# facebookarchive/Surround360

Measured on AMD Instinct MI355X. Metric: stereo-equirect frames/sec at 8K, 17-cam rig, higher is better.
Workload: dtype f32

## Files before the change

surround360_amd/csrc/flow_kernels.hip:

```cpp
#include "flow_kernels.hpp"

#include <algorithm>
#include <cmath>
#include <cstdlib>
#include <stdexcept>

#include "devmath.hpp"

namespace s360 {

typedef float f4a8 __attribute__((ext_vector_type(4), aligned(8)));

__global__ __launch_bounds__(256) void k_resize_cubic_u8c4(const uchar4* __restrict__ src, int sw, int sh,
                                                           size_t sbs, uchar4* __restrict__ dst, int dw, int dh,
                                                           size_t dbs, double scx, double scy,
                                                           const uchar4* const* __restrict__ src_tab) {
  __shared__ int s_sx[32], s_sy[8];
  __shared__ short s_ax[32][4], s_ay[8][4];
  const int tid = threadIdx.y * blockDim.x + threadIdx.x;
  if (tid < 40) {
    const bool col = tid < 32;
    const int k = col ? tid : tid - 32;
    const int d = col ? min((int)(blockIdx.x * 32 + k), dw - 1) : min((int)(blockIdx.y * 8 + k), dh - 1);
    int s0;
// ... 211 lines not shown
  for (int j = 0; j < 4; ++j) {
    int sx;
    float cb[4];
    resize_coord(min(dx0 + j, dw - 1), scx, &sx, &f);
    cubic_coeffs(f, cb);
    int a[4];
#pragma unroll
    for (int k = 0; k < 4; ++k) a[k] = sat_s16(cv_round(cb[k] * 2048.f));
    c[j] = sx - 1 - bx0;
    w01[j] = __builtin_bit_cast(s16x2, (unsigned)(a[0] & 0xffff) | ((unsigned)a[1] << 16));
    w23[j] = __builtin_bit_cast(s16x2, (unsigned)(a[2] & 0xffff) | ((unsigned)a[3] << 16));
  }
  int r0, ay[4];
  {
    int sy;
    float cb[4];
    resize_coord(min(dy, dh - 1), scy, &sy, &f);
    cubic_coeffs(f, cb);
#pragma unroll
    for (int k = 0; k < 4; ++k) ay[k] = sat_s16(cv_round(cb[k] * 2048.f));
    r0 = sy - 1 - by0;
  }
  __syncthreads();
  if (dx0 >= dw || dy >= dh) return;
  const float scale = 1.f / (2048 * 2048);
  const float b0 = (float)ay[0] * scale, b1 = (float)ay[1] * scale, b2 = (float)ay[2] * scale, b3 = (float)ay[3] * scale;
  auto pixel = [&](int j, const unsigned (&p)[4][4]) -> unsigned {
    const bool sse = dx0 + j < (dw & ~1);
    unsigned o = 0;
#pragma unroll
    for (int ch = 0; ch < 4; ++ch) {
      const unsigned sel = 0x0c040c00u + ch * 0x00010001u;
      int hh[4];
#pragma unroll
      for (int r = 0; r < 4; ++r) {
        const s16x2 lo = __builtin_bit_cast(s16x2, __builtin_amdgcn_perm(p[r][1], p[r][0], sel));
        const s16x2 hi = __builtin_bit_cast(s16x2, __builtin_amdgcn_perm(p[r][3], p[r][2], sel));
        hh[r] = __builtin_amdgcn_sdot2(lo, w01[j], 0, false);
        hh[r] = __builtin_amdgcn_sdot2(hi, w23[j], hh[r], false);
      }
      int v;
      if (sse) {
        float s = (float)hh[0] * b0;
        s = s + (float)hh[1] * b1;
        s = s + (float)hh[2] * b2;
        s = s + (float)hh[3] * b3;
        v = cv_round(s);
      } else {
        v = (__mul24(hh[0], ay[0]) + __mul24(hh[1], ay[1]) + __mul24(hh[2], ay[2]) + __mul24(hh[3], ay[3]) + (1 << 21)) >> 22;
      }
      o |= (unsigned)sat_u8(v) << (8 * ch);
    }
    return o;
  };
  unsigned o[4];
  if (c[1] == c[0] + 2 && c[2] == c[0] + 4 && c[3] == c[0] + 6 && (c[0] & 3) == 0) {
    unsigned t[4][10];
#pragma unroll
    for (int r = 0; r < 4; ++r) {
      const unsigned* row = &s_box[r0 + r][c[0]];
      const u32x4 q0 = *reinterpret_cast<const u32x4*>(row), q1 = *reinterpret_cast<const u32x4*>(row + 4);
      typedef unsigned u32x2 __attribute__((ext_vector_type(2)));
      const u32x2 q2 = *reinterpret_cast<const u32x2*>(row + 8);
      t[r][0] = q0.x; t[r][1] = q0.y; t[r][2] = q0.z; t[r][3] = q0.w;
      t[r][4] = q1.x; t[r][5] = q1.y; t[r][6] = q1.z; t[r][7] = q1.w;
      t[r][8] = q2.x; t[r][9] = q2.y;
    }
#pragma unroll
    for (int j = 0; j < 4; ++j) {
      unsigned p[4][4];
#pragma unroll
      for (int r = 0; r < 4; ++r)
#pragma unroll
        for (int k = 0; k < 4; ++k) p[r][k] = t[r][2 * j + k];
      o[j] = pixel(j, p);
    }
  } else {
#pragma unroll
    for (int j = 0; j < 4; ++j) {
      unsigned p[4][4];
#pragma unroll
      for (int r = 0; r < 4; ++r)
#pragma unroll
        for (int k = 0; k < 4; ++k) p[r][k] = s_box[r0 + r][c[j] + k];
      o[j] = pixel(j, p);
    }
  }
  const size_t off = (size_t)dy * dw + dx0;
  const bool whole = dx0 + 3 < dw;
  if (dst) {
    unsigned* Dr = reinterpret_cast<unsigned*>(dst + dbs * blockIdx.z) + off;
    if (whole) {
      *reinterpret_cast<u32x4a4*>(Dr) = u32x4a4{o[0], o[1], o[2], o[3]};
    } else {
#pragma unroll
      for (int j = 0; j < 4; ++j)
        if (dx0 + j < dw) Dr[j] = o[j];
    }
  }
  if (gray) {
    const float inv255 = (float)(1.0 / 255.0);
    float g[4], a[4];
#pragma unroll
    for (int j = 0; j < 4; ++j) {
      const int gi = (int)((o[j] & 0xff) * 1868 + ((o[j] >> 8) & 0xff) * 9617 + ((o[j] >> 16) & 0xff) * 4899 + (1 << 13)) >> 14;
      g[j] = (float)gi * inv255;
      a[j] = (float)(o[j] >> 24) * inv255;
    }
    float* Gr = gray + pbs * blockIdx.z + off;
    float* Ar = alpha + pbs * blockIdx.z + off;
    if (whole) {
      *reinterpret_cast<f32x4a4*>(Gr) = f32x4a4{g[0], g[1], g[2], g[3]};
      *reinterpret_cast<f32x4a4*>(Ar) = f32x4a4{a[0], a[1], a[2], a[3]};
    } else {
#pragma unroll
      for (int j = 0; j < 4; ++j)
        if (dx0 + j < dw) { Gr[j] = g[j]; Ar[j] = a[j]; }
    }
  }
}

__global__ __launch_bounds__(256) void k_gray_alpha(const uchar4* __restrict__ src, size_t n, size_t sbs,
                                                    float* __restrict__ gray, float* __restrict__ alpha,
                                                    size_t pbs) {
  const size_t i = (size_t)blockIdx.x * blockDim.x + threadIdx.x;
  if (i >= n) return;
  const uchar4 p = src[sbs * blockIdx.z + i];
  const float inv255 = (float)(1.0 / 255.0);
  const int g = (p.x * 1868 + p.y * 9617 + p.z * 4899 + (1 << 13)) >> 14;
  gray[pbs * blockIdx.z + i] = (float)g * inv255;
  alpha[pbs * blockIdx.z + i] = (float)p.w * inv255;
}

__global__ __launch_bounds__(256) void k_motion(const uchar4* __restrict__ cur, const uchar4* __restrict__ prev,
                                                size_t n, size_t sbs, float* __restrict__ motion, size_t pbs) {
  const size_t i = (size_t)blockIdx.x * blockDim.x + threadIdx.x;
  if (i >= n) return;
  const uchar4 a = cur[sbs * blockIdx.z + i], b = prev[sbs * blockIdx.z + i];
  const double s = fabs((double)((int)a.x - (int)b.x)) + fabs((double)((int)a.y - (int)b.y)) +
                   fabs((double)((int)a.z - (int)b.z));
  motion[pbs * blockIdx.z + i] = (float)(s / (double)(255.0f * 3.0f));
}

#ifdef S360_WAVE_EMULATION
unsigned long long g_known_stats[2];
#define S360_KSTAT(i) __atomic_fetch_add(&g_known_stats[i], 1ull, __ATOMIC_RELAXED)
#endif
struct UpSrc {
  int sw, sh;
  size_t sbs;
  double scx, scy;
  float post_scale;
};
template <int R, int CN, int EPI, int SRC, int SB_TW = 64, int SB_TH = 16, int NT = 256>
__global__ __launch_bounds__(NT) void k_sepblur(const float* __restrict__ src, float* __restrict__ dst, int w, int h,
                                                 size_t bs , BlurTaps taps,
                                                 const float* __restrict__ A, FlowIdx idx,
                                                 const float2* __restrict__ Gp, void* __restrict__ recv,
                                                 float* const* __restrict__ dst_tab, UpSrc up,
                                                 unsigned* __restrict__ rowflags, int known_result) {
  constexpr int IW = SB_TW + 2 * R, IH = SB_TH + 2 * R;
  constexpr int IWP = IW | 1;
  __shared__ __attribute__((aligned(8))) float s_in[IH][IWP][CN];
  __shared__ __attribute__((aligned(8))) float s_mid[IH][SB_TW + 1][CN];
  const int tid = threadIdx.y * blockDim.x + threadIdx.x;
  const TileId tile = xcd_tile();
  const int tx0 = tile.x * SB_TW, ty0 = tile.y * SB_TH;
  const int vecEnd = ((w * CN) / 8) * 8;
  constexpr int kColTasks = SB_TW * (SB_TH / 4);
  static_assert(EPI == 0 || kColTasks <= NT, "one column task per thread when the epilogue is prefetched");
  float pa0[4] = {0.f, 0.f, 0.f, 0.f}, pa1[4] = {0.f, 0.f, 0.f, 0.f}, pm[4] = {0.f, 0.f, 0.f, 0.f};
  float2 pg[4];
  if (EPI != 0 && tid < kColTasks) {
    const int lx = tid % SB_TW, ly0 = (tid / SB_TW) * 4, gx = tx0 + lx;
    const size_t b0 = bs * idx.i0[tile.z], b1 = bs * idx.i1[tile.z];
#pragma unroll
    for (int o = 0; o < 4; ++o) {
      const int gy = ty0 + ly0 + o;
      pg[o] = make_float2(0.f, 0.f);
      if (gx < w && gy < h) {
        const size_t off = (size_t)gy * w + gx;
        pa0[o] = A[b0 + off];
        pa1[o] = A[b1 + off];
        if (EPI == 3) pg[o] = Gp[b0 + off];
        if (EPI == 4) {
          pg[o] = Gp[bs * tile.z + off];
          pm[o] = static_cast<const float*>(recv)[b1 + off];
        }
      }
    }
  }
  src += (SRC == 2 ? up.sbs * CN : bs * (SRC == 1 ? 1 : CN)) * tile.z;
  constexpr int LW = (IW + 7) & ~7;
  constexpr bool kColumnWalk = (NT % LW) == 0;
  const int lxc = tid % LW, lyc = tid / LW;
  const int gxc = reflect101(tx0 - R + (lxc < IW ? lxc : 0), w);
  constexpr int kLdStep = kColumnWalk ? NT / LW : NT, kLdEnd = kColumnWalk ? IH : IH * IW;
  constexpr int kLdIters = (kLdEnd + kLdStep - 1) / kLdStep;
  float ld[kLdIters][CN];
#pragma unroll
  for (int it = 0; it < kLdIters; ++it) {
    const int i = min((kColumnWalk ? lyc : tid) + it * kLdStep, kLdEnd - 1);
    const int ly = kColumnWalk ? i : i / IW, lx = kColumnWalk ? min(lxc, IW - 1) : i - ly * IW;
    const int gy = reflect101(ty0 - R + ly, h), gx = kColumnWalk ? gxc : reflect101(tx0 - R + lx, w);
    if (SRC == 2) {
      int sx, sy;
      float fx, fy;
      resize_coord(gx, up.scx, &sx, &fx);
      if (sx < 0) { fx = 0; sx = 0; }
      if (sx >= up.sw - 1) { fx = 0; sx = up.sw - 1; }
      resize_coord(gy, up.scy, &sy, &fy);
      const float* S0 = src + (size_t)clip_idx(sy, up.sh) * up.sw * CN;
      const float* S1 = src + (size_t)clip_idx(sy + 1, up.sh) * up.sw * CN;
      const float b0 = 1.f - fy, b1 = fy;
#pragma unroll
      for (int k = 0; k < CN; ++k) {
        float h0, h1;
        if (sx >= up.sw - 1) {
          h0 = S0[sx * CN + k] * 1.0f;
          h1 = S1[sx * CN + k] * 1.0f;
        } else {
          const float a0 = 1.f - fx, a1 = fx;
          h0 = S0[sx * CN + k] * a0 + S0[(sx + 1) * CN + k] * a1;
          h1 = S1[sx * CN + k] * a0 + S1[(sx + 1) * CN + k] * a1;
        }
        float v = h0 * b0 + h1 * b1;
        v *= up.post_scale;
        ld[it][k] = v;
      }
    } else if (SRC == 1) {
      const float* r0 = src + (size_t)gy * w;
      ld[it][0] = r0[min(gx + 1, w - 1)] - r0[max(gx - 1, 0)];
      ld[it][CN - 1] = src[(size_t)min(gy + 1, h - 1) * w + gx] - src[(size_t)max(gy - 1, 0) * w + gx];
    } else if (CN == 2) {
      const float2 v = *reinterpret_cast<const float2*>(src + ((size_t)gy * w + gx) * CN);
      ld[it][0] = v.x;
      ld[it][CN - 1] = v.y;
    } else {
      ld[it][0] = src[(size_t)gy * w + gx];
    }
  }
#pragma unroll
  for (int it = 0; it < kLdIters; ++it) {
    const int i = (kColumnWalk ? lyc : tid) + it * kLdStep;
    if (i >= kLdEnd || (kColumnWalk && lxc >= IW)) continue;
    const int ly = kColumnWalk ? i : i / IW, lx = kColumnWalk ? lxc : i - ly * IW;
    if (CN == 2) *reinterpret_cast<float2*>(&s_in[ly][lx][0]) = make_float2(ld[it][0], ld[it][CN - 1]);
    else s_in[ly][lx][0] = ld[it][0];
  }
  if constexpr (EPI == 2 || EPI == 3) {
    __shared__ int s_vote[NT / 64];
    bool none = true;
#pragma unroll
    for (int o = 0; o < 4; ++o) none &= !(pa0[o] > 0.9f && pa1[o] > 0.9f);
    s_vote[tid >> 6] = __ballot(!none) == 0ull;
    __syncthreads();
    int v = known_result != 0;
#pragma unroll
    for (int q = 0; q < NT / 64; ++q) v &= s_vote[q];
    const bool known = __builtin_amdgcn_readfirstlane(v) != 0;
#ifdef S360_WAVE_EMULATION
    if (tid == 0) S360_KSTAT(known ? 0 : 1);
#endif
    if (known) {
      if (tid < kColTasks) {
        const int lx = tid % SB_TW, ly0 = (tid / SB_TW) * 4, gx = tx0 + lx;
#pragma unroll
        for (int o = 0; o < 4; ++o) {
          const int gy = ty0 + ly0 + o;
          if (gx >= w || gy >= h) continue;
          const size_t off = (size_t)gy * w + gx;
          if (EPI == 2) static_cast<float2*>(recv)[bs * tile.z + off] = make_float2(__int_as_float(0x7fc00000), 0.0f);
          else static_cast<float4*>(recv)[bs * tile.z + off] = make_float4(__int_as_float(0x7fc00000), pg[o].y, 0.0f, 0.0f);
        }
      }
      return;
    }
  } else {
    __syncthreads();
  }
  for (int t = tid; t < IH * (SB_TW / 4); t += NT) {
    const int ly = t % IH, lx0 = (t / IH) * 4;
    float v[CN][4 + 2 * R];
#pragma unroll
    for (int j = 0; j < 4 + 2 * R; ++j) {
      if (CN == 2) {
        const float2 p = *reinterpret_cast<const float2*>(&s_in[ly][lx0 + j][0]);
        v[0][j] = p.x;
        v[CN - 1][j] = p.y;
      } else {
        v[0][j] = s_in[ly][lx0 + j][0];
      }
    }
#pragma unroll
    for (int o = 0; o < 4; ++o) {
      float acc[CN];
#pragma unroll
      for (int k = 0; k < CN; ++k) {
        if (R <= 2) {
          acc[k] = taps.k[0] * v[k][o + R];
#pragma unroll
          for (int j = 1; j <= R; ++j) acc[k] += taps.k[j] * (v[k][o + R + j] + v[k][o + R - j]);
        } else {
          acc[k] = ((tx0 + lx0 + o) * CN + k < vecEnd) ? 0.0f : -0.0f;
#pragma unroll
          for (int j = 0; j <= 2 * R; ++j) acc[k] += taps.k[j < R ? R - j : j - R] * v[k][o + j];
        }
      }
      if (CN == 2) *reinterpret_cast<float2*>(&s_mid[ly][lx0 + o][0]) = make_float2(acc[0], acc[CN - 1]);
      else s_mid[ly][lx0 + o][0] = acc[0];
    }
  }
  __syncthreads();
  dst = dst_tab ? dst_tab[tile.z] : dst + bs * CN * tile.z;
  for (int t = tid; t < SB_TW * (SB_TH / 4); t += NT) {
    const int lx = t % SB_TW, ly0 = (t / SB_TW) * 4;
    const int gx = tx0 + lx;
    float outv[4][CN];
    {
      float v[CN][4 + 2 * R];
#pragma unroll
      for (int j = 0; j < 4 + 2 * R; ++j) {
        if (CN == 2) {
          const float2 p = *reinterpret_cast<const float2*>(&s_mid[ly0 + j][lx][0]);
          v[0][j] = p.x;
          v[CN - 1][j] = p.y;
        } else {
          v[0][j] = s_mid[ly0 + j][lx][0];
        }
      }
      if (CN == 2) {
        typedef float f32x2 __attribute__((ext_vector_type(2)));
        f32x2 p[4 + 2 * R];
#pragma unroll
        for (int j = 0; j < 4 + 2 * R; ++j) p[j] = f32x2{v[0][j], v[CN - 1][j]};
#pragma unroll
        for (int o = 0; o < 4; ++o) {
          f32x2 acc = taps.k[0] * p[o + R] + 0.0f;
#pragma unroll
          for (int j = 1; j <= R; ++j) acc += taps.k[j] * (p[o + R + j] + p[o + R - j]);
          outv[o][0] = acc.x;
          outv[o][CN - 1] = acc.y;
        }
      } else {
#pragma unroll
        for (int k = 0; k < CN; ++k)
#pragma unroll
          for (int o = 0; o < 4; ++o) {
            float acc = taps.k[0] * v[k][o + R] + 0.0f;
#pragma unroll
            for (int j = 1; j <= R; ++j) acc += taps.k[j] * (v[k][o + R + j] + v[k][o + R - j]);
            outv[o][k] = acc;
          }
      }
    }
    if (gx >= w) continue;
#pragma unroll
    for (int o = 0; o < 4; ++o) {
      const int gy = ty0 + ly0 + o;
      if (gy >= h) continue;
      const size_t off = (size_t)gy * w + gx;
      if (EPI == 1 || EPI == 4) {
        const float cc = 1.0f - pa0[o] * pa1[o];
#pragma unroll
        for (int k = 0; k < CN; ++k) outv[o][k] = cc * outv[o][k] + (1.0f - cc) * s_in[ly0 + o + R][lx + R][k];
      }
      if (EPI == 4) {
        const float wgt = 1.0f - pm[o];
        const float px = pg[o].x * up.post_scale, py = pg[o].y * up.post_scale;
        outv[o][0] = outv[o][0] * (1.0f - wgt) + px * wgt;
        outv[o][CN - 1] = outv[o][CN - 1] * (1.0f - wgt) + py * wgt;
      }
      if (EPI == 2 || EPI == 3) {
        const bool upd = pa0[o] > 0.9f && pa1[o] > 0.9f;
        if (EPI == 2)
          static_cast<float2*>(recv)[bs * tile.z + off] = make_float2(upd ? outv[o][0] : __int_as_float(0x7fc00000), outv[o][CN - 1]);
        else
          static_cast<float4*>(recv)[bs * tile.z + off] = make_float4(upd ? pg[o].x : __int_as_float(0x7fc00000), pg[o].y, outv[o][0], outv[o][CN - 1]);
        if (rowflags && upd) rowflags[(size_t)tile.z * h + gy] = 0u;
      } else {
#pragma unroll
        for (int k = 0; k < CN; ++k) dst[off * CN + k] = outv[o][k];
      }
    }
  }
}

constexpr int UB_TW = 64, UB_TH = 16, UB_IW = UB_TW + 2, UB_IH = UB_TH + 2, UB_IWP = UB_IW | 1, UB_BW = 40, UB_BH = 14;
constexpr int UB_IN_FLOATS = UB_IH * UB_IWP * 2, UB_MID_FLOATS = UB_IH * (UB_TW + 1) * 2, UB_H_FLOATS = UB_BH * UB_IW * 2;
static_assert(UB_BH * UB_BW * 2 <= UB_IN_FLOATS, "the source box shares the input tile's storage");
static_assert(UB_H_FLOATS + 2 * UB_IW + 3 * UB_IH <= UB_MID_FLOATS, "horizontal pass + tables share the row-pass result's storage");
bool upscale_blur_tiled_fits(int sw, int sh, int dw, int dh) {
  const double scx = 1.0 / ((double)dw / (double)sw), scy = 1.0 / ((double)dh / (double)sh);
  return 2 * (long long)dw <= 5 * (long long)sw && 2 * (long long)dh <= 5 * (long long)sh && (int)std::ceil((UB_IW - 1) * scx) + 3 <= UB_BW && (int)std::ceil((UB_IH - 1) * scy) + 3 <= UB_BH;
}
__global__ __launch_bounds__(256) void k_upscale_blur_tiled(const float2* __restrict__ src, float* __restrict__ dst, int w, int h,
                                                            size_t bs, BlurTaps taps, float* const* __restrict__ dst_tab,
                                                            UpSrc up) {
  __shared__ __attribute__((aligned(16))) float s_raw[UB_IN_FLOATS + UB_MID_FLOATS];
  float2(*s_in)[UB_IWP] = reinterpret_cast<float2(*)[UB_IWP]>(s_raw);
  float2(*s_mid)[UB_TW + 1] = reinterpret_cast<float2(*)[UB_TW + 1]>(s_raw + UB_IN_FLOATS);
  float2(*s_box)[UB_BW] = reinterpret_cast<float2(*)[UB_BW]>(s_raw);
  float2(*s_h)[UB_IW] = reinterpret_cast<float2(*)[UB_IW]>(s_raw + UB_IN_FLOATS);
  int* s_sx = reinterpret_cast<int*>(s_raw + UB_IN_FLOATS + UB_H_FLOATS);
  float* s_fx = reinterpret_cast<float*>(s_sx + UB_IW);
  int* s_r0 = s_sx + 2 * UB_IW;
  int* s_r1 = s_r0 + UB_IH;
  float* s_fy = reinterpret_cast<float*>(s_r1 + UB_IH);
  const int tid = threadIdx.x;
  const TileId tile = xcd_tile();
  const int tx0 = tile.x * UB_TW, ty0 = tile.y * UB_TH;
  const int nvx = min(UB_TW, w - tx0), nvy = min(UB_TH, h - ty0);
  src += up.sbs * tile.z;
  if (tid < UB_IW) {
    int sx;
    float fx;
    resize_coord(reflect101(tx0 - 1 + min(tid, nvx + 1), w), up.scx, &sx, &fx);
    if (sx < 0) { fx = 0; sx = 0; }
    if (sx >= up.sw - 1) { fx = 0; sx = up.sw - 1; }
    s_sx[tid] = sx;
    s_fx[tid] = fx;
  } else if (tid >= 128 && tid < 128 + UB_IH) {
    const int ly = tid - 128;
    int sy;
    float fy;
    resize_coord(reflect101(ty0 - 1 + min(ly, nvy + 1), h), up.scy, &sy, &fy);
    s_r0[ly] = clip_idx(sy, up.sh);
    s_r1[ly] = clip_idx(sy + 1, up.sh);
    s_fy[ly] = fy;
  }
  __syncthreads();
  const int bx0 = min(s_sx[0], s_sx[1]), by0 = min(s_r0[0], s_r0[1]);
  const int bx1 = min(max(s_sx[nvx], s_sx[nvx + 1]) + 1, up.sw - 1), by1 = max(s_r1[nvy], s_r1[nvy + 1]);
  const int nbw = clip_idx(bx1 - bx0, UB_BW) + 1, nbh = clip_idx(by1 - by0, UB_BH) + 1;
  {
    constexpr int kIters = (UB_BW * UB_BH + 255) / 256;
    float2 ld[kIters];
#pragma unroll
    for (int it = 0; it < kIters; ++it) {
      const int i = tid + it * 256;
      const int r = min(i / UB_BW, nbh - 1), c = min(i % UB_BW, nbw - 1);
      ld[it] = src[(size_t)min(by0 + r, up.sh - 1) * up.sw + min(bx0 + c, up.sw - 1)];
    }
#pragma unroll
    for (int it = 0; it < kIters; ++it) {
      const int i = tid + it * 256;
      const int r = i / UB_BW, c = i % UB_BW;
      if (r < nbh && c < nbw) s_box[r][c] = ld[it];
    }
  }
  __syncthreads();
  for (int t = tid; t < nbh * UB_IW; t += 256) {
    const int r = t / UB_IW, c = t - r * UB_IW;
    const int sx = s_sx[c], cx = clip_idx(sx - bx0, UB_BW);
    const float2 p0 = s_box[r][cx];
    float2 hv;
    if (sx >= up.sw - 1) {
      hv.x = p0.x * 1.0f;
      hv.y = p0.y * 1.0f;
    } else {
      const float fx = s_fx[c];
      const float a0 = 1.f - fx, a1 = fx;
      const float2 p1 = s_box[r][min(cx + 1, UB_BW - 1)];
      hv.x = p0.x * a0 + p1.x * a1;
      hv.y = p0.y * a0 + p1.y * a1;
    }
    s_h[r][c] = hv;
  }
  __syncthreads();
  for (int t = tid; t < UB_IH * UB_IW; t += 256) {
    const int ly = t / UB_IW, lx = t - ly * UB_IW;
    const float fy = s_fy[ly];
    const float b0 = 1.f - fy, b1 = fy;
    const float2 h0 = s_h[clip_idx(s_r0[ly] - by0, UB_BH)][lx], h1 = s_h[clip_idx(s_r1[ly] - by0, UB_BH)][lx];
    float vx = h0.x * b0 + h1.x * b1, vy = h0.y * b0 + h1.y * b1;
    vx *= up.post_scale;
    vy *= up.post_scale;
    s_in[ly][lx] = make_float2(vx, vy);
  }
  __syncthreads();
  typedef float f32x2 __attribute__((ext_vector_type(2)));
  for (int t = tid; t < UB_IH * (UB_TW / 4); t += 256) {
    const int ly = t % UB_IH, lx0 = (t / UB_IH) * 4;
    float2 v[6];
#pragma unroll
    for (int j = 0; j < 6; ++j) v[j] = s_in[ly][lx0 + j];
#pragma unroll
    for (int o = 0; o < 4; ++o) {
      float2 acc;
      acc.x = taps.k[0] * v[o + 1].x;
      acc.x += taps.k[1] * (v[o + 2].x + v[o].x);
      acc.y = taps.k[0] * v[o + 1].y;
      acc.y += taps.k[1] * (v[o + 2].y + v[o].y);
      s_mid[ly][lx0 + o] = acc;
    }
  }
  __syncthreads();
  dst = dst_tab ? dst_tab[tile.z] : dst + bs * 2 * tile.z;
  {
    const int lx = tid % UB_TW, ly0 = (tid / UB_TW) * 4, gx = tx0 + lx;
    f32x2 p[6];
#pragma unroll
    for (int j = 0; j < 6; ++j) {
      const float2 q = s_mid[ly0 + j][lx];
      p[j] = f32x2{q.x, q.y};
    }
    if (gx >= w) return;
#pragma unroll
    for (int o = 0; o < 4; ++o) {
      const int gy = ty0 + ly0 + o;
      if (gy >= h) continue;
      f32x2 acc = taps.k[0] * p[o + 1] + 0.0f;
      acc += taps.k[1] * (p[o + 2] + p[o]);
      *reinterpret_cast<float2*>(dst + ((size_t)gy * w + gx) * 2) = make_float2(acc.x, acc.y);
    }
  }
}

template <int CN, int PPT>
__global__ __launch_bounds__(256) void k_resize_linear_f32(const float* __restrict__ src, int sw, int sh, size_t sbs,
                                                           float* __restrict__ dst, int dw, int dh, size_t dbs,
                                                           double scx, double scy, float post_scale, int do_scale) {
  const int dx = blockIdx.x * blockDim.x + threadIdx.x;
  const int dy = blockIdx.y * blockDim.y + threadIdx.y;
  if (dx >= dw || dy >= dh) return;
  int sx, sy;
  float fx, fy;
  resize_coord(dx, scx, &sx, &fx);
  if (sx < 0) { fx = 0; sx = 0; }
  if (sx >= sw - 1) { fx = 0; sx = sw - 1; }
  resize_coord(dy, scy, &sy, &fy);
  const size_t r0 = (size_t)clip_idx(sy, sh) * sw * CN, r1 = (size_t)clip_idx(sy + 1, sh) * sw * CN;
  const float b0 = 1.f - fy, b1 = fy;
  const bool edge = sx >= sw - 1;
  const int sx1 = edge ? sx : sx + 1;
  const float a0 = 1.f - fx, a1 = fx;
// ... 232 lines not shown
    dst[(size_t)dy * dw + dx] = o;
  }
}




__global__ void k_search_init(const float* __restrict__ I, const float* __restrict__ A, int w, int h, size_t pbs,
                              FlowIdx idx, float2* __restrict__ flow, int hint, int dist, float* __restrict__ I1eq) {
  const int b = blockIdx.x;
  const float* __restrict__ I0 = I + pbs * idx.i0[b];
  const float* __restrict__ I1 = I + pbs * idx.i1[b];
  const float* __restrict__ A0 = A + pbs * idx.i0[b];
  const float* __restrict__ A1 = A + pbs * idx.i1[b];
  flow += pbs * b;
  I1eq += pbs * b;
  __shared__ float s_ratio;
  if (threadIdx.x == 0) {
    float sumL = 0, sumR = 0;
    for (int i = 0; i < w * h; ++i) {
      const float a = A0[i] * A1[i];
      sumL += a * I0[i];
      sumR += a * I1[i];
    }
    s_ratio = sumL / sumR;
  }
  __syncthreads();
  const float ratio = s_ratio;
  for (int i = threadIdx.x; i < w * h; i += blockDim.x) I1eq[i] = I1[i] * ratio;
  __syncthreads();
  const int kRatio = 8;
  const int ortho = (dist + kRatio / 2) / kRatio;
  const int thickness = 2 * ortho + 1;
  int bx, by, bw, bh;
  if (hint == 1) { bx = 0; by = -ortho; bw = dist + 1; bh = thickness; }
  else if (hint == 2) { bx = -ortho; by = 0; bw = thickness; bh = dist + 1; }
  else if (hint == 3) { bx = -dist; by = -ortho; bw = dist + 1; bh = thickness; }
  else { bx = -ortho; by = -dist; bw = thickness; bh = dist + 1; }
  auto patchErr = [&](int i0x, int i0y, int i1x, int i1y) -> float {
    float sad = 0, alpha = 0;
    for (int dy = -2; dy <= 2; ++dy) {
      const int d0y = i0y + dy;
      if (0 <= d0y && d0y < h) {
        const int d1y = min(max(i1y + dy, 0), h - 1);
        for (int dx = -2; dx <= 2; ++dx) {
          const int d0x = i0x + dx;
          if (0 <= d0x && d0x < w) {
            const int d1x = min(max(i1x + dx, 0), w - 1);
            const float difference = I0[d0y * w + d0x] - I1eq[d1y * w + d1x];
            sad += fabsf(difference);
            alpha += A0[d0y * w + d0x] * A1[d1y * w + d1x];
          }
        }
      }
    }
    sad /= alpha;
    const float ddx = (float)(i1x - i0x), ddy = (float)(i1y - i0y);
    const float length = (float)sqrt((double)ddx * ddx + (double)ddy * ddy);
    sad *= 1 + length / dist;
    return sad;
  };
  for (int i = threadIdx.x; i < w * h; i += blockDim.x) {
    const int i0y = i / w, i0x = i - i0y * w;
    if (A0[i] > 0.9f) {
      float errorBest = 0.8f * patchErr(i0x, i0y, i0x, i0y);
      int bxb = i0x, byb = i0y;
      for (int dy = by; dy < by + bh; ++dy)
        for (int dx = bx; dx < bx + bw; ++dx) {
          const int i1x = i0x + dx, i1y = i0y + dy;
          if (0 <= i1x && i1x < w && 0 <= i1y && i1y < h) {
            const float e = patchErr(i0x, i0y, i1x, i1y);
            if (errorBest > e) { errorBest = e; bxb = i1x; byb = i1y; }
          }
        }
      flow[i] = make_float2((float)(bxb - i0x), (float)(byb - i0y));
    }
  }
}

bool known_result_enabled() {
  static const bool on = [] {
    const char* e = std::getenv("S360_KNOWN_RESULT");
    return !(e && e[0] == '0' && e[1] == 0);
  }();
  return on;
}

static inline dim3 grid2d(int w, int h, int B, dim3 blk) { return dim3((w + blk.x - 1) / blk.x, (h + blk.y - 1) / blk.y, B); }

bool resize_cubic_u8c4_tiled_fits(int sw, int sh, int dw, int dh) {
  const double scx = 1.0 / ((double)dw / (double)sw), scy = 1.0 / ((double)dh / (double)sh);
  return scx >= 1.5 && scy >= 1.5 && (int)std::ceil((std::min(dw, DS_TW) - 1) * scx) + 5 <= DS_BW &&
         (int)std::ceil((std::min(dh, DS_TH) - 1) * scy) + 5 <= DS_BH;
}
void launch_resize_cubic_u8c4_generic(hipStream_t st, const uchar4* src, int sw, int sh, size_t sbs, uchar4* dst, int dw,
                                      int dh, size_t dbs, int B, const uchar4* const* src_tab) {
  const double scx = 1.0 / ((double)dw / (double)sw), scy = 1.0 / ((double)dh / (double)sh);
  dim3 blk(32, 8);
  hipLaunchKernelGGL(k_resize_cubic_u8c4, grid2d(dw, dh, B, blk), blk, 0, st, src, sw, sh, sbs, dst, dw, dh, dbs, scx,
                     scy, src_tab);
}
void launch_resize_cubic_u8c4(hipStream_t st, const uchar4* src, int sw, int sh, size_t sbs, uchar4* dst, int dw,
                              int dh, size_t dbs, int B, const uchar4* const* src_tab) {
  const double scx = 1.0 / ((double)dw / (double)sw), scy = 1.0 / ((double)dh / (double)sh);
  if (sh == dh && !src_tab && known_result_enabled() && (int)std::ceil((HR_TW - 1) * scx) + 12 <= HR_BW) {
    hipLaunchKernelGGL((k_resize_cubic_u8c4_h<false, false>), dim3((dw + HR_TW - 1) / HR_TW, (dh + HR_TH - 1) / HR_TH, B), dim3(256),
                       0, st, src, sw, sh, sbs, (void*)dst, dw, dbs, scx);
    return;
  }
  if (resize_cubic_u8c4_tiled_fits(sw, sh, dw, dh)) {
    hipLaunchKernelGGL(k_resize_cubic_u8c4_tiled, dim3((dw + DS_TW - 1) / DS_TW, (dh + DS_TH - 1) / DS_TH, B), dim3(256), 0, st,
                       src, sw, sh, sbs, dst, dw, dh, dbs, scx, scy, src_tab, (float*)nullptr, (float*)nullptr, (size_t)0);
    return;
  }
  launch_resize_cubic_u8c4_generic(st, src, sw, sh, sbs, dst, dw, dh, dbs, B, src_tab);
}
bool launch_resize_cubic_u8c4_to_bgr(hipStream_t st, const uchar4* src, int sw, int sh, uint8_t* dst_bgr, int dw, int dh) {
  const double scx = 1.0 / ((double)dw / (double)sw);
  if (!(sh == dh && known_result_enabled() && (int)std::ceil((HR_TW - 1) * scx) + 12 <= HR_BW)) return false;
  const dim3 grid((dw + HR_TW - 1) / HR_TW, (dh + HR_TH - 1) / HR_TH, 1);
  if ((dw & 3) == 0 && (reinterpret_cast<uintptr_t>(dst_bgr) & 3) == 0)
    hipLaunchKernelGGL((k_resize_cubic_u8c4_h<true, true>), grid, dim3(256), 0, st, src, sw, sh, (size_t)0, (void*)dst_bgr, dw, (size_t)0, scx);
  else
    hipLaunchKernelGGL((k_resize_cubic_u8c4_h<true, false>), grid, dim3(256), 0, st, src, sw, sh, (size_t)0, (void*)dst_bgr, dw, (size_t)0, scx);
  return true;
}
void launch_entry_downscale(hipStream_t st, const uchar4* src, int sw, int sh, size_t sbs, uchar4* down, uchar4* scratch, int dw,
                            int dh, size_t dbs, int B, const uchar4* const* src_tab, float* gray, float* alpha, size_t pbs) {
  if (resize_cubic_u8c4_tiled_fits(sw, sh, dw, dh)) {
    const double scx = 1.0 / ((double)dw / (double)sw), scy = 1.0 / ((double)dh / (double)sh);
    hipLaunchKernelGGL(k_resize_cubic_u8c4_tiled, dim3((dw + DS_TW - 1) / DS_TW, (dh + DS_TH - 1) / DS_TH, B), dim3(256), 0, st,
                       src, sw, sh, sbs, down, dw, dh, dbs, scx, scy, src_tab, gray, alpha, pbs);
    return;
  }
  uchar4* d = down ? down : scratch;
  launch_resize_cubic_u8c4_generic(st, src, sw, sh, sbs, d, dw, dh, dbs, B, src_tab);
  launch_gray_alpha(st, d, (size_t)dw * dh, dbs, gray, alpha, pbs, B);
}
void launch_gray_alpha(hipStream_t st, const uchar4* src, size_t n, size_t sbs, float* gray, float* alpha, size_t pbs,
                       int B) {
  hipLaunchKernelGGL(k_gray_alpha, dim3((unsigned)((n + 255) / 256), 1, B), dim3(256), 0, st, src, n, sbs, gray, alpha,
                     pbs);
}
void launch_motion(hipStream_t st, const uchar4* cur, const uchar4* prev, size_t n, size_t sbs, float* motion,
                   size_t pbs, int B) {
  hipLaunchKernelGGL(k_motion, dim3((unsigned)((n + 255) / 256), 1, B), dim3(256), 0, st, cur, prev, n, sbs, motion,
                     pbs);
}
template <int R, int CN, int EPI, int SRC>
static void launch_sepblur_t(hipStream_t st, const float* src, float* dst, int w, int h, size_t bs, int B,
                             const BlurTaps& t, const float* A, const FlowIdx& idx, const float2* Gp, void* rec,
                             float* const* dst_tab = nullptr, const UpSrc& up = UpSrc{}, unsigned* rowflags = nullptr) {
  dim3 blk(64, 4);
  if constexpr (R == 7) {
    dim3 grd((w + 31) / 32, (h + 31) / 32, B);
    hipLaunchKernelGGL((k_sepblur<R, CN, EPI, SRC, 32, 32, 384>), grd, dim3(64, 6), 0, st, src, dst, w, h, bs, t, A, idx, Gp, rec, dst_tab, up, rowflags, known_result_enabled() ? 1 : 0);
  } else {
    dim3 grd((w + 63) / 64, (h + 15) / 16, B);
    hipLaunchKernelGGL((k_sepblur<R, CN, EPI, SRC>), grd, blk, 0, st, src, dst, w, h, bs, t, A, idx, Gp, rec, dst_tab, up, rowflags, known_result_enabled() ? 1 : 0);
  }
}
void launch_sepblur(hipStream_t st, const float* src, float* dst, int w, int h, int cn, size_t bs, int B,
                    const BlurTaps& t, float* const* dst_tab) {
  static const FlowIdx none = {nullptr, nullptr};
  if (t.r == 1 && cn == 1) launch_sepblur_t<1, 1, 0, 0>(st, src, dst, w, h, bs, B, t, nullptr, none, nullptr, nullptr);
  else if (t.r == 1 && cn == 2) launch_sepblur_t<1, 2, 0, 0>(st, src, dst, w, h, bs, B, t, nullptr, none, nullptr, nullptr, dst_tab);
  else if (t.r == 2 && cn == 1) launch_sepblur_t<2, 1, 0, 0>(st, src, dst, w, h, bs, B, t, nullptr, none, nullptr, nullptr);
  else if (t.r == 7 && cn == 2) launch_sepblur_t<7, 2, 0, 0>(st, src, dst, w, h, bs, B, t, nullptr, none, nullptr, nullptr);
  else throw std::runtime_error("launch_sepblur: unsupported radius/channels");
}
void launch_diffusion(hipStream_t st, const float2* flow, float2* dst, int w, int h, size_t bs, int B,
                      const BlurTaps& t, const float* A, const FlowIdx& idx) {
  launch_sepblur_t<7, 2, 1, 0>(st, (const float*)flow, (float*)dst, w, h, bs, B, t, A, idx, nullptr, nullptr);
}
void launch_diffusion_adjust(hipStream_t st, const float2* flow, float2* dst, int w, int h, size_t bs, int B, const BlurTaps& t,
                             const float* A, const FlowIdx& idx, const float2* prev, const float* motion, float prev_scale) {
  UpSrc up{};
  up.post_scale = prev_scale;
  launch_sepblur_t<7, 2, 4, 0>(st, (const float*)flow, (float*)dst, w, h, bs, B, t, A, idx, prev, const_cast<float*>(motion), nullptr, up);
}
void launch_upscale_blur(hipStream_t st, const float2* src, int sw, int sh, size_t sbs, float2* dst, int dw, int dh,
                         size_t dbs, int B, float post_scale, const BlurTaps& t, float* const* dst_tab, bool generic) {
  static const FlowIdx none = {nullptr, nullptr};
  if (t.r != 1) throw std::runtime_error("launch_upscale_blur: 3x3 kernel expected");
  UpSrc up;
  up.sw = sw; up.sh = sh; up.sbs = sbs;
  up.scx = 1.0 / ((double)dw / (double)sw);
  up.scy = 1.0 / ((double)dh / (double)sh);
  up.post_scale = post_scale;
  if (!generic && upscale_blur_tiled_fits(sw, sh, dw, dh))
    hipLaunchKernelGGL(k_upscale_blur_tiled, dim3((dw + UB_TW - 1) / UB_TW, (dh + UB_TH - 1) / UB_TH, B), dim3(256), 0, st, src,
                       (float*)dst, dw, dh, dbs, t, dst_tab, up);
  else
    launch_sepblur_t<1, 2, 0, 2>(st, (const float*)src, (float*)dst, dw, dh, dbs, B, t, nullptr, none, nullptr, nullptr, dst_tab, up);
}
void launch_gradients(hipStream_t st, const float* I, float2* G, int w, int h, size_t bs, int B, const BlurTaps& t) {
  static const FlowIdx none = {nullptr, nullptr};
  if (t.r != 1) throw std::runtime_error("launch_gradients: 3x3 kernel expected");
  launch_sepblur_t<1, 2, 0, 1>(st, I, (float*)G, w, h, bs, B, t, nullptr, none, nullptr, nullptr);
}
void launch_blur_to_records(hipStream_t st, const float2* flow, void* rec, int w, int h, size_t bs, int B,
                            const BlurTaps& t, const float2* G, const float* A, const FlowIdx& idx, unsigned* rowflags) {
  if (t.r != 7) throw std::runtime_error("launch_blur_to_records: 15x15 kernel expected");
  if (G) launch_sepblur_t<7, 2, 3, 0>(st, (const float*)flow, nullptr, w, h, bs, B, t, A, idx, G, rec, nullptr, UpSrc{}, rowflags);
  else launch_sepblur_t<7, 2, 2, 0>(st, (const float*)flow, nullptr, w, h, bs, B, t, A, idx, nullptr, rec, nullptr, UpSrc{}, rowflags);
}
bool resize_linear_f32_tiled(int sw, int sh, int dw, int dh, int cn) {
  const double scx = 1.0 / ((double)dw / (double)sw), scy = 1.0 / ((double)dh / (double)sh);
  const int tw = std::min(dw, RL_TW), th = std::min(dh, RL_TH);
  const bool fits = std::min(sw, (int)std::floor((tw - 1) * scx) + 3) + 3 <= RL_BW &&
                    std::min(sh, (int)std::floor((th - 1) * scy) + 3) <= RL_BH;
  return cn == 1 && fits;
}
void launch_resize_linear_f32(hipStream_t st, const float* src, int sw, int sh, size_t sbs, float* dst, int dw, int dh,
                              size_t dbs, int cn, int B, float post_scale, int do_scale) {
  const double scx = 1.0 / ((double)dw / (double)sw), scy = 1.0 / ((double)dh / (double)sh);
  const int ppt = (B % 4 == 0) ? 4 : (B % 2 == 0) ? 2 : 1;
  if (resize_linear_f32_tiled(sw, sh, dw, dh, cn)) {
    const dim3 grid((dw + RL_TW - 1) / RL_TW, (dh + RL_TH - 1) / RL_TH, B / ppt);
#define S360_RLT(P)                                                                                                   \
  hipLaunchKernelGGL((k_resize_linear_f32c1_tiled<P>), grid, dim3(256), 0, st, src, sw, sh, sbs, dst, dw, dh, dbs, scx, \
                     scy, post_scale, do_scale)
    if (ppt == 4) S360_RLT(4); else if (ppt == 2) S360_RLT(2); else S360_RLT(1);
#undef S360_RLT
    return;
  }
  dim3 blk(32, 8);
#define S360_RL(C, P)                                                                                                   \
  hipLaunchKernelGGL((k_resize_linear_f32<C, P>), grid2d(dw, dh, B / P, blk), blk, 0, st, src, sw, sh, sbs, dst, dw, dh, \
                     dbs, scx, scy, post_scale, do_scale)
  if (cn == 1) { if (ppt == 4) S360_RL(1, 4); else if (ppt == 2) S360_RL(1, 2); else S360_RL(1, 1); }
  else { if (ppt == 4) S360_RL(2, 4); else if (ppt == 2) S360_RL(2, 2); else S360_RL(2, 1); }
#undef S360_RL
}
bool resize_cubic_f32c2_tiled(int sw, int sh, int dw, int dh, bool src_tab) {
  const double scx = 1.0 / ((double)dw / (double)sw), scy = 1.0 / ((double)dh / (double)sh);
  return !src_tab && scx <= 1.0 && scy <= 1.0;
}
void launch_resize_cubic_f32c2(hipStream_t st, const float2* src, int sw, int sh, size_t sbs, float2* dst, int dw,
                               int dh, size_t dbs, int B, float post_scale, const float2* const* src_tab) {
  const double scx = 1.0 / ((double)dw / (double)sw), scy = 1.0 / ((double)dh / (double)sh);
  if (resize_cubic_f32c2_tiled(sw, sh, dw, dh, src_tab != nullptr)) {
    hipLaunchKernelGGL(k_resize_cubic_f32c2_tiled, dim3((dw + UC_TW - 1) / UC_TW, (dh + UC_TH - 1) / UC_TH, B), dim3(256),
                       0, st, src, sw, sh, sbs, dst, dw, dh, dbs, scx, scy, post_scale);
    return;
  }
  dim3 blk(32, 8);
  hipLaunchKernelGGL(k_resize_cubic_f32c2, grid2d(dw, dh, B, blk), blk, 0, st, src, sw, sh, sbs, dst, dw, dh, dbs, scx,
                     scy, post_scale, src_tab);
}
void launch_search_init(hipStream_t st, const float* I, const float* A, int w, int h, size_t pbs, int B,
                        const FlowIdx& idx, float2* flow, int hint, int dist, float* I1eq) {
  hipLaunchKernelGGL(k_search_init, dim3(B), dim3(256), 0, st, I, A, w, h, pbs, idx, flow, hint, dist, I1eq);
}

}
```

Baseline: 53.32.

## Use 32-bit plane offsets in sepblur and add tiled gradients kernel

Templates the separable blur kernel on a WIDE flag so that, when plane sizes fit in 31 bits, per-pixel addressing uses 32-bit offsets (mul24 plus incremental row strides) in place of 64-bit size_t arithmetic. It also writes the CN=2 output as a single float2 store and precomputes the shared-memory store address for the column walk. A new dedicated gradients kernel loads an aligned float4 grey box into LDS, computes central differences from there, then blurs with 3x3 taps, replacing the generic sepblur SRC=1 path that did four scattered global loads per pixel. The cost is more template instantiations, an environment switch for the tiled path, and extra alignment and boundary logic that must reproduce reflect101 exactly.

New measurement: 53.82 (median of 6 runs). About the same (+0.9%).

```diff
diff --git a/surround360_amd/csrc/flow_kernels.hip b/surround360_amd/csrc/flow_kernels.hip
--- a/surround360_amd/csrc/flow_kernels.hip
+++ b/surround360_amd/csrc/flow_kernels.hip
@@ -387,7 +387,34 @@
   double scx, scy;
   float post_scale;
 };
-template <int R, int CN, int EPI, int SRC, int SB_TW = 64, int SB_TH = 16, int NT = 256>
+template <class T>
+__device__ __forceinline__ T ld_off32(const void* base, unsigned byte_off) {
+  return *reinterpret_cast<const T*>(static_cast<const char*>(base) + byte_off);
+}
+template <bool WIDE>
+struct PlaneOff {
+  typedef unsigned type;
+  static __device__ __forceinline__ unsigned at(int y, int w, int x) { return (unsigned)(__mul24(y, w) + x); }
+  template <class T>
+  static __device__ __forceinline__ T ld(const T* base, unsigned i) { return ld_off32<T>(base, i * (unsigned)sizeof(T)); }
+  template <class T>
+  static __device__ __forceinline__ void st(T* base, unsigned i, const T& v) {
+    *reinterpret_cast<T*>(reinterpret_cast<char*>(base) + i * (unsigned)sizeof(T)) = v;
+  }
+};
+template <>
+struct PlaneOff<true> {
+  typedef size_t type;
+  static __device__ __forceinline__ size_t at(int y, int w, int x) { return (size_t)y * w + x; }
+  template <class T>
+  static __device__ __forceinline__ T ld(const T* base, size_t i) { return base[i]; }
+  template <class T>
+  static __device__ __forceinline__ void st(T* base, size_t i, const T& v) { base[i] = v; }
+};
+inline bool plane_offsets_fit_32(int w, int h, size_t widest_element) {
+  return w < (1 << 23) && h < (1 << 23) && (unsigned long long)w * (unsigned long long)h * widest_element < (1ull << 31);
+}
+template <int R, int CN, int EPI, int SRC, int SB_TW = 64, int SB_TH = 16, int NT = 256, bool WIDE = false>
 __global__ __launch_bounds__(NT) void k_sepblur(const float* __restrict__ src, float* __restrict__ dst, int w, int h,
                                                  size_t bs , BlurTaps taps,
                                                  const float* __restrict__ A, FlowIdx idx,
@@ -406,21 +433,33 @@
   static_assert(EPI == 0 || kColTasks <= NT, "one column task per thread when the epilogue is prefetched");
   float pa0[4] = {0.f, 0.f, 0.f, 0.f}, pa1[4] = {0.f, 0.f, 0.f, 0.f}, pm[4] = {0.f, 0.f, 0.f, 0.f};
   float2 pg[4];
+  typedef PlaneOff<WIDE> PO;
+  typedef typename PO::type off_t;
+  const float* A0 = A;
+  const float* A1 = A;
+  const float2* Gb = Gp;
+  const float* Mb = static_cast<const float*>(recv);
+  if (EPI != 0) {
+    const size_t b0 = bs * idx.i0[tile.z], b1 = bs * idx.i1[tile.z];
+    A0 += b0;
+    A1 += b1;
+    if (EPI == 3) Gb += b0;
+    if (EPI == 4) { Gb += bs * tile.z; Mb += b1; }
+  }
   if (EPI != 0 && tid < kColTasks) {
     const int lx = tid % SB_TW, ly0 = (tid / SB_TW) * 4, gx = tx0 + lx;
-    const size_t b0 = bs * idx.i0[tile.z], b1 = bs * idx.i1[tile.z];
-#pragma unroll
-    for (int o = 0; o < 4; ++o) {
+    off_t off = PO::at(ty0 + ly0, w, gx);
+#pragma unroll
+    for (int o = 0; o < 4; ++o, off += (off_t)w) {
       const int gy = ty0 + ly0 + o;
       pg[o] = make_float2(0.f, 0.f);
       if (gx < w && gy < h) {
-        const size_t off = (size_t)gy * w + gx;
-        pa0[o] = A[b0 + off];
-        pa1[o] = A[b1 + off];
-        if (EPI == 3) pg[o] = Gp[b0 + off];
+        pa0[o] = PO::ld(A0, off);
+        pa1[o] = PO::ld(A1, off);
+        if (EPI == 3) pg[o] = PO::ld(Gb, off);
         if (EPI == 4) {
-          pg[o] = Gp[bs * tile.z + off];
-          pm[o] = static_cast<const float*>(recv)[b1 + off];
+          pg[o] = PO::ld(Gb, off);
+          pm[o] = PO::ld(Mb, off);
         }
       }
     }
@@ -464,15 +503,15 @@
         ld[it][k] = v;
       }
     } else if (SRC == 1) {
-      const float* r0 = src + (size_t)gy * w;
-      ld[it][0] = r0[min(gx + 1, w - 1)] - r0[max(gx - 1, 0)];
-      ld[it][CN - 1] = src[(size_t)min(gy + 1, h - 1) * w + gx] - src[(size_t)max(gy - 1, 0) * w + gx];
+      const off_t r0 = PO::at(gy, w, 0);
+      ld[it][0] = PO::ld(src, r0 + (off_t)min(gx + 1, w - 1)) - PO::ld(src, r0 + (off_t)max(gx - 1, 0));
+      ld[it][CN - 1] = PO::ld(src, PO::at(min(gy + 1, h - 1), w, gx)) - PO::ld(src, PO::at(max(gy - 1, 0), w, gx));
     } else if (CN == 2) {
-      const float2 v = *reinterpret_cast<const float2*>(src + ((size_t)gy * w + gx) * CN);
+      const float2 v = PO::ld(reinterpret_cast<const float2*>(src), PO::at(gy, w, gx));
       ld[it][0] = v.x;
       ld[it][CN - 1] = v.y;
     } else {
-      ld[it][0] = src[(size_t)gy * w + gx];
+      ld[it][0] = PO::ld(src, PO::at(gy, w, gx));
     }
   }
 #pragma unroll
@@ -480,8 +519,9 @@
     const int i = (kColumnWalk ? lyc : tid) + it * kLdStep;
     if (i >= kLdEnd || (kColumnWalk && lxc >= IW)) continue;
     const int ly = kColumnWalk ? i : i / IW, lx = kColumnWalk ? lxc : i - ly * IW;
-    if (CN == 2) *reinterpret_cast<float2*>(&s_in[ly][lx][0]) = make_float2(ld[it][0], ld[it][CN - 1]);
-    else s_in[ly][lx][0] = ld[it][0];
+    float* const d = kColumnWalk ? &s_in[0][0][0] + (lyc * IWP + lxc) * CN + it * (kLdStep * IWP * CN) : &s_in[ly][lx][0];
+    if (CN == 2) *reinterpret_cast<float2*>(d) = make_float2(ld[it][0], ld[it][CN - 1]);
+    else d[0] = ld[it][0];
   }
   if constexpr (EPI == 2 || EPI == 3) {
     __shared__ int s_vote[NT / 64];
@@ -500,13 +540,15 @@
     if (known) {
       if (tid < kColTasks) {
         const int lx = tid % SB_TW, ly0 = (tid / SB_TW) * 4, gx = tx0 + lx;
-#pragma unroll
-        for (int o = 0; o < 4; ++o) {
+        float2* const rec2 = static_cast<float2*>(recv) + bs * tile.z;
+        float4* const rec4 = static_cast<float4*>(recv) + bs * tile.z;
+        off_t off = PO::at(ty0 + ly0, w, gx);
+#pragma unroll
+        for (int o = 0; o < 4; ++o, off += (off_t)w) {
           const int gy = ty0 + ly0 + o;
           if (gx >= w || gy >= h) continue;
-          const size_t off = (size_t)gy * w + gx;
-          if (EPI == 2) static_cast<float2*>(recv)[bs * tile.z + off] = make_float2(__int_as_float(0x7fc00000), 0.0f);
-          else static_cast<float4*>(recv)[bs * tile.z + off] = make_float4(__int_as_float(0x7fc00000), pg[o].y, 0.0f, 0.0f);
+          if (EPI == 2) PO::st(rec2, off, make_float2(__int_as_float(0x7fc00000), 0.0f));
+          else PO::st(rec4, off, make_float4(__int_as_float(0x7fc00000), pg[o].y, 0.0f, 0.0f));
         }
       }
       return;
@@ -590,11 +632,14 @@
       }
     }
     if (gx >= w) continue;
-#pragma unroll
-    for (int o = 0; o < 4; ++o) {
+    float2* const rec2 = static_cast<float2*>(recv) + bs * tile.z;
+    float4* const rec4 = static_cast<float4*>(recv) + bs * tile.z;
+    unsigned* const flags = rowflags ? rowflags + (size_t)tile.z * h : nullptr;
+    off_t off = PO::at(ty0 + ly0, w, gx);
+#pragma unroll
+    for (int o = 0; o < 4; ++o, off += (off_t)w) {
       const int gy = ty0 + ly0 + o;
       if (gy >= h) continue;
-      const size_t off = (size_t)gy * w + gx;
       if (EPI == 1 || EPI == 4) {
         const float cc = 1.0f - pa0[o] * pa1[o];
 #pragma unroll
@@ -609,14 +654,118 @@
       if (EPI == 2 || EPI == 3) {
         const bool upd = pa0[o] > 0.9f && pa1[o] > 0.9f;
         if (EPI == 2)
-          static_cast<float2*>(recv)[bs * tile.z + off] = make_float2(upd ? outv[o][0] : __int_as_float(0x7fc00000), outv[o][CN - 1]);
+          PO::st(rec2, off, make_float2(upd ? outv[o][0] : __int_as_float(0x7fc00000), outv[o][CN - 1]));
         else
-          static_cast<float4*>(recv)[bs * tile.z + off] = make_float4(upd ? pg[o].x : __int_as_float(0x7fc00000), pg[o].y, outv[o][0], outv[o][CN - 1]);
-        if (rowflags && upd) rowflags[(size_t)tile.z * h + gy] = 0u;
+          PO::st(rec4, off, make_float4(upd ? pg[o].x : __int_as_float(0x7fc00000), pg[o].y, outv[o][0], outv[o][CN - 1]));
+        if (rowflags && upd) PO::st(flags, (off_t)gy, 0u);
+      } else if (CN == 2) {
+        PO::st(reinterpret_cast<float2*>(dst), off, make_float2(outv[o][0], outv[o][CN - 1]));
       } else {
-#pragma unroll
-        for (int k = 0; k < CN; ++k) dst[off * CN + k] = outv[o][k];
-      }
+        PO::st(dst, off, outv[o][0]);
+      }
+    }
+  }
+}
+
+constexpr int GT_TW = 64, GT_TH = 16, GT_IW = GT_TW + 2, GT_IH = GT_TH + 2, GT_IWP = GT_IW | 1;
+constexpr int GT_BH = GT_TH + 4, GT_PAD = 3, GT_PIECES = (GT_TW + 4 + GT_PAD + 3) / 4, GT_BW = 4 * GT_PIECES + 4;
+constexpr int GT_IN_FLOATS = GT_IH * GT_IWP * 2, GT_MID_FLOATS = GT_IH * (GT_TW + 1) * 2;
+static_assert(GT_BH * GT_BW + 4 * GT_IH <= GT_MID_FLOATS, "the grey box and the row table share the row-pass result's storage");
+static_assert(GT_PAD + 4 * (GT_PIECES - 1) + 3 < GT_BW, "the last piece of a row ends inside the box's row");
+__global__ __launch_bounds__(256) void k_gradients_tiled(const float* __restrict__ I, float2* __restrict__ G, int w, int h,
+                                                         size_t bs, BlurTaps taps) {
+  typedef float f32x2 __attribute__((ext_vector_type(2)));
+  typedef float f32x4 __attribute__((ext_vector_type(4)));
+  __shared__ __attribute__((aligned(16))) float s_raw[GT_IN_FLOATS + GT_MID_FLOATS];
+  f32x2(*s_in)[GT_IWP] = reinterpret_cast<f32x2(*)[GT_IWP]>(s_raw);
+  f32x2(*s_mid)[GT_TW + 1] = reinterpret_cast<f32x2(*)[GT_TW + 1]>(s_raw + GT_IN_FLOATS);
+  float(*s_box)[GT_BW] = reinterpret_cast<float(*)[GT_BW]>(s_raw + GT_IN_FLOATS);
+  int(*s_rows)[4] = reinterpret_cast<int(*)[4]>(s_raw + GT_IN_FLOATS + GT_BH * GT_BW);
+  const int tid = threadIdx.x;
+  const TileId tile = xcd_tile();
+  const int tx0 = tile.x * GT_TW, ty0 = tile.y * GT_TH;
+  const float* const P = I + bs * tile.z;
+  const int bx0 = max(tx0 - 2, 0), by0 = max(ty0 - 2, 0);
+  const int nbw = min(tx0 + GT_TW + 2, w) - bx0, nbh = min(ty0 + GT_TH + 2, h) - by0;
+  {
+    const int mis = (int)((reinterpret_cast<uintptr_t>(P) >> 2) & 3u);
+    const int last = w * h - 1;
+    constexpr int kIters = (GT_BH * GT_PIECES + 255) / 256;
+    f32x4 ld[kIters];
+    int col[kIters];
+#pragma unroll
+    for (int it = 0; it < kIters; ++it) {
+      const int i = tid + it * 256, ri = i / GT_PIECES, k = i - ri * GT_PIECES;
+      const int r = min(ri, nbh - 1);
+      const int e = (by0 + r) * w + bx0;
+      const int a = (mis + e) & 3;
+      const int kk = min(k, (nbw - 1 + a) >> 2);
+      const int pe = e - a + 4 * kk;
+      col[it] = (ri < nbh && k == kk) ? GT_PAD - a + 4 * k : -1;
+      if (pe >= 0 && pe + 3 <= last) {
+        ld[it] = ld_off32<f32x4>(P, (unsigned)pe * 4u);
+      } else {
+        ld[it] = f32x4{ld_off32<float>(P, (unsigned)clip_idx(pe, last + 1) * 4u), ld_off32<float>(P, (unsigned)clip_idx(pe + 1, last + 1) * 4u),
+                       ld_off32<float>(P, (unsigned)clip_idx(pe + 2, last + 1) * 4u), ld_off32<float>(P, (unsigned)clip_idx(pe + 3, last + 1) * 4u)};
+      }
+    }
+#pragma unroll
+    for (int it = 0; it < kIters; ++it) {
+      if (col[it] < 0) continue;
+      float* d = &s_box[min((tid + it * 256) / GT_PIECES, GT_BH - 1)][col[it]];
+      d[0] = ld[it].x; d[1] = ld[it].y; d[2] = ld[it].z; d[3] = ld[it].w;
+    }
+  }
+  if (tid < GT_IH) {
+    const int pr = min(ty0 - 1 + tid, h);
+    const int r = clip_idx(pr < 0 ? -pr : pr >= h ? 2 * h - 2 - pr : pr, h);
+    s_rows[tid][0] = clip_idx(r - by0, nbh) * GT_BW;
+    s_rows[tid][1] = clip_idx(max(r - 1, 0) - by0, nbh) * GT_BW;
+    s_rows[tid][2] = clip_idx(min(r + 1, h - 1) - by0, nbh) * GT_BW;
+  }
+  __syncthreads();
+  if (tid < 3 * GT_IW) {
+    const int lr = tid / GT_IW, lx = tid - lr * GT_IW;
+    const int pc = min(tx0 - 1 + lx, w);
+    const int c = clip_idx(pc < 0 ? -pc : pc >= w ? 2 * w - 2 - pc : pc, w);
+    const int bc = clip_idx(c - bx0, nbw) + GT_PAD;
+    const int bl = clip_idx(max(c - 1, 0) - bx0, nbw) + GT_PAD, br = clip_idx(min(c + 1, w - 1) - bx0, nbw) + GT_PAD;
+    const float* const box = &s_box[0][0];
+#pragma unroll
+    for (int it = 0; it < GT_IH / 3; ++it) {
+      const int ly = lr + 3 * it;
+      const int rc = s_rows[ly][0], ru = s_rows[ly][1], rd = s_rows[ly][2];
+      s_in[ly][lx] = f32x2{box[rc + br] - box[rc + bl], box[rd + bc] - box[ru + bc]};
+    }
+  }
+  __syncthreads();
+  for (int t = tid; t < GT_IH * (GT_TW / 4); t += 256) {
+    const int ly = t % GT_IH, lx0 = (t / GT_IH) * 4;
+    f32x2 v[6];
+#pragma unroll
+    for (int j = 0; j < 6; ++j) v[j] = s_in[ly][lx0 + j];
+#pragma unroll
+    for (int o = 0; o < 4; ++o) {
+      f32x2 acc = taps.k[0] * v[o + 1];
+      acc += taps.k[1] * (v[o + 2] + v[o]);
+      s_mid[ly][lx0 + o] = acc;
+    }
+  }
+  __syncthreads();
+  {
+    const int lx = tid % GT_TW, ly0 = (tid / GT_TW) * 4, gx = tx0 + lx, gy0 = ty0 + ly0;
+    f32x2 p[6];
+#pragma unroll
+    for (int j = 0; j < 6; ++j) p[j] = s_mid[ly0 + j][lx];
+    if (gx >= w) return;
+    char* const D = reinterpret_cast<char*>(G + bs * tile.z);
+    unsigned off = ((unsigned)gy0 * (unsigned)w + (unsigned)gx) * 8u;
+#pragma unroll
+    for (int o = 0; o < 4; ++o, off += (unsigned)w * 8u) {
+      if (gy0 + o >= h) break;
+      f32x2 acc = taps.k[0] * p[o + 1] + 0.0f;
+      acc += taps.k[1] * (p[o + 2] + p[o]);
+      *reinterpret_cast<f32x2*>(D + off) = acc;
     }
   }
 }
@@ -1155,12 +1304,20 @@
                              const BlurTaps& t, const float* A, const FlowIdx& idx, const float2* Gp, void* rec,
                              float* const* dst_tab = nullptr, const UpSrc& up = UpSrc{}, unsigned* rowflags = nullptr) {
   dim3 blk(64, 4);
+  const bool narrow = plane_offsets_fit_32(w, h, EPI == 3 ? 16 : 8);
+  const int kr = known_result_enabled() ? 1 : 0;
   if constexpr (R == 7) {
     dim3 grd((w + 31) / 32, (h + 31) / 32, B);
-    hipLaunchKernelGGL((k_sepblur<R, CN, EPI, SRC, 32, 32, 384>), grd, dim3(64, 6), 0, st, src, dst, w, h, bs, t, A, idx, Gp, rec, dst_tab, up, rowflags, known_result_enabled() ? 1 : 0);
+    if (narrow)
+      hipLaunchKernelGGL((k_sepblur<R, CN, EPI, SRC, 32, 32, 384, false>), grd, dim3(64, 6), 0, st, src, dst, w, h, bs, t, A, idx, Gp, rec, dst_tab, up, rowflags, kr);
+    else
+      hipLaunchKernelGGL((k_sepblur<R, CN, EPI, SRC, 32, 32, 384, true>), grd, dim3(64, 6), 0, st, src, dst, w, h, bs, t, A, idx, Gp, rec, dst_tab, up, rowflags, kr);
   } else {
     dim3 grd((w + 63) / 64, (h + 15) / 16, B);
-    hipLaunchKernelGGL((k_sepblur<R, CN, EPI, SRC>), grd, blk, 0, st, src, dst, w, h, bs, t, A, idx, Gp, rec, dst_tab, up, rowflags, known_result_enabled() ? 1 : 0);
+    if (narrow)
+      hipLaunchKernelGGL((k_sepblur<R, CN, EPI, SRC, 64, 16, 256, false>), grd, blk, 0, st, src, dst, w, h, bs, t, A, idx, Gp, rec, dst_tab, up, rowflags, kr);
+    else
+      hipLaunchKernelGGL((k_sepblur<R, CN, EPI, SRC, 64, 16, 256, true>), grd, blk, 0, st, src, dst, w, h, bs, t, A, idx, Gp, rec, dst_tab, up, rowflags, kr);
   }
 }
 void launch_sepblur(hipStream_t st, const float* src, float* dst, int w, int h, int cn, size_t bs, int B,
@@ -1200,6 +1357,12 @@
 void launch_gradients(hipStream_t st, const float* I, float2* G, int w, int h, size_t bs, int B, const BlurTaps& t) {
   static const FlowIdx none = {nullptr, nullptr};
   if (t.r != 1) throw std::runtime_error("launch_gradients: 3x3 kernel expected");
+  const char* e = std::getenv("S360_GRADIENTS_TILED");
+  const bool off = e && e[0] == '0' && e[1] == 0;
+  if (!off && plane_offsets_fit_32(w, h, 8)) {
+    hipLaunchKernelGGL(k_gradients_tiled, dim3((w + GT_TW - 1) / GT_TW, (h + GT_TH - 1) / GT_TH, B), dim3(256), 0, st, I, G, w, h, bs, t);
+    return;
+  }
   launch_sepblur_t<1, 2, 0, 1>(st, I, (float*)G, w, h, bs, B, t, nullptr, none, nullptr, nullptr);
 }
 void launch_blur_to_records(hipStream_t st, const float2* flow, void* rec, int w, int h, size_t bs, int B,
```
